# AnyDSL/rodent

Measured on AMD Instinct MI355X. Metric: Mrays/s, higher is better.
Workload: dtype f32; 1 GPU; atrium.bvh + atrium-primary.rays (1024x1024 primary rays, tmax 5000, closest hit); bvh_layout=BVH2, kernel=k_bvh2_top_auto<false,15, 255, 16, 32>, variant=top, parallelism=replicated BVH x 1, world_size=1

## Files before the change

include/rodent_traversal.h:

```cpp
#ifndef RODENT_TRAVERSAL_H
#define RODENT_TRAVERSAL_H

#include <stdint.h>
#include <stddef.h>

#ifdef __cplusplus
extern "C" {
#endif


struct Node2 {
    float   bounds[12];
    int32_t child[2];
    int32_t pad[2];
};

struct Tri1 {
    float   v0[3];  int32_t pad;
    float   e1[3];  int32_t geom_id;
    float   e2[3];  int32_t prim_id;
};

struct Node4 {
    float   bounds[6][4];
// ... 46 lines not shown
void hip_traverse_bvh2_tri1_async(int32_t dev,
        const struct Node2* nodes, const struct Tri1* tris,
        const struct Ray1* rays, struct Hit1* hits, int32_t num_rays,
        int32_t any_hit, int32_t variant, void* stream);
void hip_traverse_bvh4_tri4_async(int32_t dev,
        const struct Node4* nodes, const struct Tri4* tris,
        const struct Ray1* rays, struct Hit1* hits, int32_t num_rays,
        int32_t any_hit, int32_t variant, void* stream);
void hip_traverse_bvh8_tri4_async(int32_t dev,
        const struct Node8* nodes, const struct Tri4* tris,
        const struct Ray1* rays, struct Hit1* hits, int32_t num_rays,
        int32_t any_hit, int32_t variant, void* stream);
int32_t rodent_hip_check_errors(int32_t dev, void* stream);

uint64_t    rodent_hip_get_kernel_time(void);
int32_t     rodent_hip_device_count(void);
int32_t     rodent_hip_num_variants(int32_t bvh_width);
void        rodent_hip_phased_min_rays(int32_t rays);
void        rodent_hip_top_min_rays(int32_t rays);
void        rodent_hip_schedule_history(int32_t enable);
void        rodent_hip_ray_kind_hint(int32_t enable);
void        rodent_hip_ray_grid(int32_t width);
void        rodent_hip_octant_loops(int32_t enable);
int32_t     rodent_hip_is_lab_build(void);
const char* rodent_hip_variant_name(int32_t bvh_width, int32_t variant);
const char* rodent_hip_kernel_name(int32_t bvh_width, int32_t variant, int32_t any_hit);
const char* rodent_hip_version(void);
const char* rodent_hip_source_digest(void);
void        rodent_hip_read_stats(int32_t dev, uint64_t* out8);
void        rodent_hip_read_trace(int32_t dev, uint64_t* out);
void        rodent_hip_debug_set_perm(int32_t dev, const int32_t* device_perm);

#ifdef __cplusplus
}
#endif
#endif
```

rodent_amd/abi.py:

```python
from __future__ import annotations

import ctypes as C
import os
from pathlib import Path

import numpy as np
import torch

from . import formats as F

LAB = os.environ.get("RODENT_HIP_LAB", "0") not in ("", "0")
LIB_PATH = Path(__file__).resolve().parent / "lib" / ("librodent_hip_lab.so" if LAB else "librodent_hip.so")
if os.environ.get("RODENT_HIP_LIB"):
    LIB_PATH = Path(os.environ["RODENT_HIP_LIB"]).resolve()

SYNC_ENTRY_POINTS = [
    "amdgpu_intersect_single_ray1_bvh2_tri1", "amdgpu_occluded_single_ray1_bvh2_tri1",
    "hip_intersect_single_ray1_bvh4_tri4", "hip_occluded_single_ray1_bvh4_tri4",
    "hip_intersect_single_ray1_bvh8_tri4", "hip_occluded_single_ray1_bvh8_tri4",
]
ASYNC_ENTRY_POINTS = ["hip_traverse_bvh2_tri1_async", "hip_traverse_bvh4_tri4_async", "hip_traverse_bvh8_tri4_async"]
EXPORTS = SYNC_ENTRY_POINTS + ASYNC_ENTRY_POINTS + [
    "rodent_hip_check_errors", "rodent_hip_get_kernel_time", "rodent_hip_device_count", "rodent_hip_num_variants",
        "rodent_hip_variant_name",
    "rodent_hip_kernel_name", "rodent_hip_version", "rodent_hip_source_digest", "rodent_hip_is_lab_build", "rodent_hip_phased_min_rays",
        "rodent_hip_top_min_rays", "rodent_hip_ray_kind_hint", "rodent_hip_ray_grid", "rodent_hip_octant_loops", "rodent_hip_schedule_history",
        "rodent_hip_read_stats", "rodent_hip_read_trace", "rodent_hip_debug_set_perm",
    "rodent_hip_build_scratch_bytes", "rodent_hip_build_bvh2_tri1", "rodent_hip_build_bvh2_tri1_sync",
    "rodent_hip_build_opt_scratch_bytes", "rodent_hip_build_bvh2_tri1_opt", "rodent_hip_build_bvh2_tri1_opt_sync",
    "rodent_hip_build_split_max_refs", "rodent_hip_build_split_scratch_bytes", "rodent_hip_build_bvh2_tri1_split",
    "rodent_hip_build_bvh2_tri1_split_sync",
    "rodent_hip_refit_scratch_bytes", "rodent_hip_refit_bvh2_tri1", "rodent_hip_refit_bvh2_tri1_sync",
    "rodent_hip_refit_wide_scratch_bytes", "rodent_hip_refit_bvh4_tri4", "rodent_hip_refit_bvh4_tri4_sync",
    "rodent_hip_refit_bvh8_tri4", "rodent_hip_refit_bvh8_tri4_sync",
    "rodent_hip_collapse_scratch_bytes", "rodent_hip_collapse_bvh2_tri1", "rodent_hip_collapse_bvh2_tri1_sync",
    "rodent_hip_collapse_bounded_scratch_bytes", "rodent_hip_collapse_bvh2_tri1_bounded", "rodent_hip_collapse_bvh2_tri1_bounded_sync",
]
BLOCK_OF_WIDTH = {2: F.BVH2_TRI1, 4: F.BVH4_TRI4, 8: F.BVH8_TRI4}

_lib = None


class BuildOptions(C.Structure):
    _fields_ = [("max_leaf", C.c_int32), ("treelet_passes", C.c_int32), ("node_cost", C.c_float), ("tri_cost", C.c_float)]


class SplitOptions(C.Structure):
    _fields_ = [("budget", C.c_float), ("max_pieces", C.c_int32)]

# ... 1 lines not shown
class MissingExtension(RuntimeError):
    pass


def lib():
    global _lib
    if _lib is None:
        if not LIB_PATH.exists():
            raise MissingExtension(f"{LIB_PATH} not built: run `python -m rodent_amd.build` (needs hipcc)")
        l = C.CDLL(str(LIB_PATH))
        vp, i32 = C.c_void_p, C.c_int32
        for name in SYNC_ENTRY_POINTS:
            fn = getattr(l, name); fn.restype = None; fn.argtypes = [i32, vp, vp, vp, vp, i32]
        for name in ASYNC_ENTRY_POINTS:
            fn = getattr(l, name); fn.restype = None; fn.argtypes = [i32, vp, vp, vp, vp, i32, i32, i32, vp]
        l.rodent_hip_check_errors.restype = i32; l.rodent_hip_check_errors.argtypes = [i32, vp]
        l.rodent_hip_is_lab_build.restype = i32; l.rodent_hip_is_lab_build.argtypes = []
        l.rodent_hip_phased_min_rays.restype = None; l.rodent_hip_phased_min_rays.argtypes = [i32]
        l.rodent_hip_top_min_rays.restype = None; l.rodent_hip_top_min_rays.argtypes = [i32]
        l.rodent_hip_get_kernel_time.restype = C.c_uint64; l.rodent_hip_get_kernel_time.argtypes = []
        l.rodent_hip_ray_kind_hint.restype = None; l.rodent_hip_ray_kind_hint.argtypes = [i32]
        l.rodent_hip_ray_grid.restype = None; l.rodent_hip_ray_grid.argtypes = [i32]
        l.rodent_hip_octant_loops.restype = None; l.rodent_hip_octant_loops.argtypes = [i32]
        l.rodent_hip_schedule_history.restype = None; l.rodent_hip_schedule_history.argtypes = [i32]
        l.rodent_hip_device_count.restype = i32; l.rodent_hip_device_count.argtypes = []
        l.rodent_hip_num_variants.restype = i32; l.rodent_hip_num_variants.argtypes = [i32]
        l.rodent_hip_variant_name.restype = C.c_char_p; l.rodent_hip_variant_name.argtypes = [i32, i32]
        l.rodent_hip_kernel_name.restype = C.c_char_p; l.rodent_hip_kernel_name.argtypes = [i32, i32, i32]
        l.rodent_hip_version.restype = C.c_char_p; l.rodent_hip_version.argtypes = []
        l.rodent_hip_source_digest.restype = C.c_char_p; l.rodent_hip_source_digest.argtypes = []
        l.rodent_hip_read_trace.restype = None; l.rodent_hip_read_trace.argtypes = [i32, C.c_void_p]
        l.rodent_hip_debug_set_perm.restype = None; l.rodent_hip_debug_set_perm.argtypes = [i32, C.c_void_p]
        l.rodent_hip_read_stats.restype = None; l.rodent_hip_read_stats.argtypes = [i32, C.POINTER(C.c_uint64)]
        l.rodent_hip_build_scratch_bytes.restype = C.c_int64; l.rodent_hip_build_scratch_bytes.argtypes = [i32]
        l.rodent_hip_build_bvh2_tri1.restype = i32
        l.rodent_hip_build_bvh2_tri1.argtypes = [i32, vp, i32, vp, i32, i32, vp, vp, vp, vp, vp]
        l.rodent_hip_build_bvh2_tri1_sync.restype = i32
        l.rodent_hip_build_bvh2_tri1_sync.argtypes = [i32, vp, i32, vp, i32, i32, vp, vp, C.POINTER(i32)]
        opt = C.POINTER(BuildOptions)
        l.rodent_hip_build_opt_scratch_bytes.restype = C.c_int64; l.rodent_hip_build_opt_scratch_bytes.argtypes = [i32, opt]
        l.rodent_hip_build_bvh2_tri1_opt.restype = i32
        l.rodent_hip_build_bvh2_tri1_opt.argtypes = [i32, vp, i32, vp, i32, opt, vp, vp, vp, vp, vp]
        l.rodent_hip_build_bvh2_tri1_opt_sync.restype = i32
        l.rodent_hip_build_bvh2_tri1_opt_sync.argtypes = [i32, vp, i32, vp, i32, opt, vp, vp, C.POINTER(i32)]
        spl = C.POINTER(SplitOptions)
        l.rodent_hip_build_split_max_refs.restype = C.c_int64; l.rodent_hip_build_split_max_refs.argtypes = [i32, spl]
# ... 45 lines not shown


def kernel_name(width, variant, any_hit=False):
    return lib().rodent_hip_kernel_name(width, variant, int(any_hit)).decode()



def to_device(arr: np.ndarray, dev: int = 0):
    import torch
    if not torch.cuda.is_available():
        raise RuntimeError("rodent_amd: no GPU visible (torch.cuda.is_available() is False)")
    a = np.ascontiguousarray(arr)
    t = torch.from_numpy(a.view(np.uint8).reshape(-1).copy() if a.size else np.zeros(0, np.uint8))
    return t.to(f"cuda:{dev}")


def from_device(t, dtype: np.dtype) -> np.ndarray:
    return t.cpu().numpy().view(dtype).copy()


class DeviceBvh:

    def __init__(self, width, nodes, tris, dev=0):
        assert width in (2, 4, 8)
        self.width, self.dev = width, dev
        self.num_nodes, self.num_tris = len(nodes), len(tris)
        self.nodes = to_device(nodes, dev)
        self.tris = to_device(tris, dev)

    @classmethod
    def from_tensors(cls, width, nodes, tris, num_nodes, num_tris, dev=0):
        assert width in (2, 4, 8)
        node_dt, tri_dt = {2: (F.NODE2, F.TRI1), 4: (F.NODE4, F.TRI4), 8: (F.NODE8, F.TRI4)}[width]
        for t, count, dt in ((nodes, num_nodes, node_dt), (tris, num_tris, tri_dt)):
            if not t.is_cuda or t.numel() * t.element_size() < count * dt.itemsize or not t.is_contiguous():
                raise ValueError("DeviceBvh.from_tensors: a contiguous CUDA tensor with room for every record is needed")
        self = cls.__new__(cls)
        self.width, self.dev = width, dev
        self.num_nodes, self.num_tris = int(num_nodes), int(num_tris)
        self.nodes, self.tris = nodes, tris
        return self

    @classmethod
    def load(cls, path, width, dev=0):
        nodes, tris = F.read_bvh(path, BLOCK_OF_WIDTH[width])
        return cls(width, nodes, tris, dev)


def traverse_async(bvh: DeviceBvh, rays_dev, hits_dev, num_rays, any_hit=False, variant=0, stream=None):
    import torch
    if stream is None:
# ... 23 lines not shown
    return from_device(hits_dev, F.HIT1)[:n]


def schedule_history(enable: bool):
    lib().rodent_hip_schedule_history(int(bool(enable)))


def top_min_rays(rays: int):
    lib().rodent_hip_top_min_rays(int(rays))


def ray_kind_hint(enable: bool):
    lib().rodent_hip_ray_kind_hint(int(bool(enable)))


def ray_grid(width: int = -1):
    lib().rodent_hip_ray_grid(int(width))


def octant_loops(enable: bool = True):
    lib().rodent_hip_octant_loops(int(bool(enable)))


def check_errors(dev=0, stream=None):
    import torch
    if stream is None:
        stream = torch.cuda.current_stream(dev)
    if lib().rodent_hip_check_errors(dev, C.c_void_p(stream.cuda_stream)):
        raise RuntimeError("rodent_hip: traversal stack overflow (more than 64 entries)")


def read_stats(dev=0):
    buf = (C.c_uint64 * 8)()
    lib().rodent_hip_read_stats(dev, buf)
    return list(buf)


def read_trace(dev=0, arm_only=False):
    if arm_only:
        lib().rodent_hip_read_trace(dev, None)
        return None
    buf = np.zeros((16384, 4), np.uint64)
    lib().rodent_hip_read_trace(dev, buf.ctypes.data_as(C.c_void_p))
    return buf
```

rodent_amd/csrc/traversal.hip:

```cpp
#include <hip/hip_runtime.h>

#include <algorithm>
#include <atomic>
#include <cstdint>
#include <cstdio>
#include <cstdlib>
#include <memory>
#include <mutex>
#include <utility>
#include <vector>

#include "device_buffer.h"
#include "rodent_traversal.h"
#include "traversal_device.h"

namespace {

using namespace rodent_dev;

template <bool ANY, bool WIDE = true>
__device__ __forceinline__ bool leaf_tri1(const Tri1* __restrict__ tris, int first, RayX& ray, HitAcc& hit) {
    int j = first;
    for (;;) {
        const float4* p = WIDE ? reinterpret_cast<const float4*>(tris + j)
// ... 85 lines not shown
            report_error(ctl);
        }
    }
}

template <bool ANY>
__global__ __launch_bounds__(kWave) void k_bvh2_finish(const Node2* __restrict__ nodes, const Tri1* __restrict__ tris,
                                                        const Ray1* __restrict__ rays, Hit1* __restrict__ hits,
                                                        Ctl* ctl, const int* __restrict__ deep_list,
                                                            int* , int* phase_counters) {
    __shared__ int stack_lds[kStackCap * kWave];
    finish_launch<ANY>(nodes, tris, rays, hits, ctl, deep_list, (lds_int*)stack_lds, phase_counters, blockIdx.x, gridDim.x);
}

struct Lane {
    RayX ray;
    int top;
    lds_int* sp;
    int ray_id;
    bool found;
};
typedef const __attribute__((address_space(1))) char* gptr;
struct Bases { gptr node, tri; };
__device__ __forceinline__ Bases make_bases(const Node2* nodes, const Tri1* tris) {
    unsigned long long node_bits = reinterpret_cast<unsigned long long>(nodes - 1), tri_bits = reinterpret_cast<unsigned long long>(tris);
    asm volatile("" : "+v"(node_bits), "+v"(tri_bits));
    return Bases{(gptr)node_bits, (gptr)tri_bits};
}

typedef __attribute__((address_space(3))) float lds_float;
template <bool ANY, bool PF = false, bool TOP = false, bool LAZY = false, bool FENCE = false, bool SHARED = false, int SPILL = 0,
    int WPG = 1, int OCT = -1>
__device__ __forceinline__ void bvh2_step(Lane& L, const Bases& base, Hit1* __restrict__ hits, lds_int* sp_limit, Ctl* ctl,
    int* __restrict__ deep_list,
                                          bool prefetch = false, lds_int* pf_row = nullptr, lds_int* image = nullptr,
                                              lds_float* shared_tmax = nullptr,
                                          int* __restrict__ spill = nullptr, const RaySplat* splat = nullptr) {
    const bool is_node = L.top > 0;
    typedef float f32x4 __attribute__((ext_vector_type(4)));
    typedef int i32x2 __attribute__((ext_vector_type(2)));
    f32x4 q0, q1, q2;
    i32x2 ch;
    int popped;
    float shared_now = 0.0f;
    if constexpr (TOP && !SHARED) {
        const unsigned idx = (unsigned)(is_node ? L.top : ~L.top), stride = is_node ? (unsigned)sizeof(Node2) : (unsigned)sizeof(Tri1);
        const gptr addr = (is_node ? base.node : base.tri) + (size_t)idx * stride;
        joint_fetch(q0, q1, q2, ch, popped, L.top >= kLdsTag, (unsigned)(size_t)image + (unsigned)(L.top - kLdsTag), addr,
            addr + (is_node ? 48u : 40u), L.sp);
    } else {
        if (TOP && L.top >= kLdsTag) {
            typedef __attribute__((address_space(3))) const char* lds_bytes;
            const lds_bytes rec = (lds_bytes)image + (unsigned)(L.top - kLdsTag);
            const __attribute__((address_space(3))) f32x4* p = (const __attribute__((address_space(3))) f32x4*)rec;
            q0 = p[0]; q1 = p[1]; q2 = p[2];
            ch = *(const __attribute__((address_space(3))) i32x2*)(rec + 48);
        } else {
            const unsigned idx = (unsigned)(is_node ? L.top : ~L.top), stride = is_node ? (unsigned)sizeof(Node2) : (unsigned)sizeof(Tri1);
            const gptr addr = (is_node ? base.node : base.tri) + (size_t)idx * stride;
            const __attribute__((address_space(1))) f32x4* p = (const __attribute__((address_space(1))) f32x4*)addr;
            q0 = p[0]; q1 = p[1]; q2 = p[2];
            ch = *(const __attribute__((address_space(1))) i32x2*)(addr + (is_node ? 48u : 40u));
        }
        popped = *L.sp;
        if (SHARED) shared_now = *shared_tmax;
        asm volatile("" : "+v"(q0), "+v"(q1), "+v"(q2), "+v"(ch));
    }
    if (SHARED) {
// ... 445 lines not shown
    int want = 64;
    while (want < slots) want *= 2;
    s.spill.ensure((size_t)std::min(want, kSpillSlots) * kSpillWaveInts);
}
int persistent_groups(const DeviceState& s, int occ, int waves) {
    const int groups = ((s.num_cus * (occ / waves) + kStripes - 1) / kStripes) * kStripes;
    if ((long)groups * waves > kSpillSlots) {
        fprintf(stderr, "rodent_hip: %d x %d resident waves exceed the %d stack spill blocks\n", groups, waves, kSpillSlots); abort(); }
    return groups;
}

bool read_and_clear_error_flags(DeviceState& s, hipStream_t stream) {
    HIP_CHECK(hipStreamSynchronize(stream));
    volatile int* page = s.host_page;
    const bool raised = page[kHostErr] != 0;
    page[kHostErr] = 0;
    return raised;
}
void check_error_flag(DeviceState& s, hipStream_t stream) {
    if (read_and_clear_error_flags(s, stream)) {
        fprintf(stderr, "rodent_hip: traversal stack overflow (more than %d entries)\n", kStackCap); abort(); }
}

int mapped_node_ids(const Node2* nodes) {
    hipDeviceptr_t range_base = nullptr; size_t range_size = 0;
    if (hipMemGetAddressRange(&range_base, &range_size, (hipDeviceptr_t)nodes) != hipSuccess) { (void)hipGetLastError(); return 0; }
    const size_t bytes = (size_t)((const char*)range_base + range_size - (const char*)nodes);
    return (int)std::min<size_t>(bytes / sizeof(Node2), 0x3FFFFFFF);
}

int g_ray_grid = [] { const char* e = getenv("RODENT_HIP_RAY_GRID"); return e ? atoi(e) : -1; }();
int g_octant_loops = [] { const char* e = getenv("RODENT_HIP_OCTANT_LOOPS"); return e ? (atoi(e) ? 1 : 0) : 1; }();
int g_schedule_history = [] { const char* e = getenv("RODENT_HIP_SCHEDULE_HISTORY"); return e && atoi(e) ? 1 : 0; }();
constexpr int kFinishGroups = 256;
#define LAUNCH_ARGS DeviceState& s, const Node2* nodes, const Tri1* tris, const Ray1* rays, Hit1* hits, int n, hipStream_t stream

constexpr int kGridMinRays = 2048 * kWave;
bool reserve_single(DeviceState& s, int n, bool spill) {
    s.deep_list.ensure(n);
    spill = spill && blocks_for(n) <= kSpillSlots;
    if (spill) ensure_spill(s, blocks_for(n));
    return spill;
}
template <bool ANY, int LDS_N, int XCD, bool TR = false, int PRIO = 0> void L_single(LAUNCH_ARGS) {
    if (reserve_single(s, n, PRIO == 0 && !TR))
        hipLaunchKernelGGL((k_bvh2_single<ANY, LDS_N, XCD, false, 0, true>), dim3(blocks_for(n)), dim3(kWave), 0, stream, nodes, tris,
            rays, hits, n, s.ctl(), s.deep_list.ptr, (const int*)nullptr, s.spill.ptr, n >= kGridMinRays ? g_ray_grid : 0);
    else
        hipLaunchKernelGGL((k_bvh2_single<ANY, LDS_N, XCD, TR, PRIO>), dim3(blocks_for(n)), dim3(kWave), 0, stream, nodes, tris, rays,
            hits, n, s.ctl(), s.deep_list.ptr, (const int*)nullptr, (int*)nullptr, 0);
    hipLaunchKernelGGL((k_bvh2_finish<ANY>), dim3(kFinishGroups), dim3(kWave), 0, stream, nodes, tris, rays, hits, s.ctl(),
        s.deep_list.ptr, s.deep_stack, (int*)nullptr);
// ... 68 lines not shown
}
template <bool ANY, int LDS_N, int TOPN, int WAVES, int REFILL, int MODE = 0, bool FUSED = true,
    bool LAZY = false> void L_default(LAUNCH_ARGS) {
    const int max_id = reserve_default(s, nodes, n, WAVES);
    if (max_id == 0) { L_single<ANY, 16, 32>(s, nodes, tris, rays, hits, n, stream); return; }
    if (g_schedule_history) {
        launch_top_persist<ANY, LDS_N, TOPN, WAVES, false, false, 32, false, 0, 2>(s, nodes, tris, rays, hits, n, stream, max_id); return; }
    const int groups = persistent_groups(s, 32, WAVES);
    s.top_image_nodes = nullptr; s.order_rays = 0;
    if (s.hint_rays != rays || s.hint_n != n) { s.hint_rays = rays; s.hint_n = n; s.hint_first_id = s.launch_id + 1; }
    const int id = ++s.launch_id;
    const volatile int* kinds = s.host_kinds;
    const bool hinting = MODE == 0 && g_kind_hint;
    int* const report_to = hinting ? s.host_kinds : nullptr;
    const bool incoherent = hinting && kinds[1] >= s.hint_first_id && kinds[0] < kinds[1];
    if (incoherent) {
        hipLaunchKernelGGL((k_bvh2_top_refill<ANY, LDS_N, TOPN, WAVES, REFILL, false, false>), dim3(groups), dim3(kWave * WAVES), 0,
            stream, nodes, tris, rays, hits, n, s.ctl(), s.deep_list.ptr,
                           (const int4*)s.top_image.ptr, s.tickets.ptr, max_id, s.spill.ptr, report_to, id);
        hipLaunchKernelGGL((k_bvh2_top_finish<ANY>), dim3(1), dim3(kWave), 0, stream, nodes, tris, rays, hits, s.ctl(), s.deep_list.ptr,
            s.deep_stack, s.tickets.ptr, s.top_image.ptr, TOPN);
        return;
    }
    hipLaunchKernelGGL((k_bvh2_top_auto<ANY, LDS_N, TOPN, WAVES, REFILL, MODE, FUSED, LAZY>), dim3(groups), dim3(kWave * WAVES), 0, stream,
        nodes, tris, rays, hits, n, s.ctl(), s.deep_list.ptr,
                       s.top_image.ptr, s.tickets.ptr, max_id, s.spill.ptr, report_to, id, g_ray_grid, g_octant_loops);
    if (!FUSED) hipLaunchKernelGGL((k_bvh2_top_finish<ANY>), dim3(1), dim3(kWave), 0, stream, nodes, tris, rays, hits, s.ctl(),
        s.deep_list.ptr, s.deep_stack, s.tickets.ptr, s.top_image.ptr, TOPN);
}

template <bool ANY, int LDS_N, int TOPN, int WAVES, int REFILL, bool ADAPT = false, bool FENCE = false> void L_top_refill(LAUNCH_ARGS) {
    if (top_kernel_ids(nodes, n) == 0) { L_single<ANY, 16, 32>(s, nodes, tris, rays, hits, n, stream); return; }
    const int groups = persistent_groups(s, 32, WAVES);
    s.deep_list.ensure(n);
    ensure_top_buffers(s);
    s.top_image_nodes = nullptr;
    ensure_spill(s, groups * WAVES);
    hipLaunchKernelGGL((k_bvh2_top_refill<ANY, LDS_N, TOPN, WAVES, REFILL, ADAPT, FENCE>), dim3(groups), dim3(kWave * WAVES), 0, stream,
        nodes, tris, rays, hits, n, s.ctl(), s.deep_list.ptr,
                       (const int4*)s.top_image.ptr, s.tickets.ptr, mapped_node_ids(nodes), s.spill.ptr, (int*)nullptr, 0);
    hipLaunchKernelGGL((k_bvh2_top_finish<ANY>), dim3(1), dim3(kWave), 0, stream, nodes, tris, rays, hits, s.ctl(), s.deep_list.ptr,
        s.deep_stack, s.tickets.ptr, s.top_image.ptr, TOPN);
}



template <bool ANY, int LDS_N> void L_sorted(LAUNCH_ARGS) {
    s.deep_list.ensure(n);
    ensure_sort_buffers(s, n);
// ... 195 lines not shown
    timed_sync_call(dev, num_rays, nullptr,
        [&](DeviceState& s) { launch_wide(8, false, s, nodes, tris, rays, hits, num_rays, default_variant(8), nullptr); });
}
void hip_occluded_single_ray1_bvh8_tri4(int32_t dev, const Node8* nodes, const Tri4* tris, const Ray1* rays, Hit1* hits, int32_t num_rays) {
    timed_sync_call(dev, num_rays, nullptr,
        [&](DeviceState& s) { launch_wide(8, true, s, nodes, tris, rays, hits, num_rays, default_variant(8), nullptr); });
}

int32_t rodent_hip_device_count(void) {
    int count = 0;
    if (hipGetDeviceCount(&count) != hipSuccess) return 0;
    return count;
}
int32_t rodent_hip_num_variants(int32_t bvh_width) {
    if (bvh_width == 2) return kNumVariants2;
    int count = 0; wide_variants(bvh_width, &count); return count;
}
const char* rodent_hip_variant_name(int32_t bvh_width, int32_t variant) {
    if (bvh_width == 2) return variant >= 0 && variant < kNumVariants2 ? kVariants2[variant].name : "";
    int count = 0; const VariantW* t = wide_variants(bvh_width, &count);
    return variant >= 0 && variant < count ? t[variant].name : "";
}
const char* rodent_hip_kernel_name(int32_t bvh_width, int32_t variant, int32_t any_hit) {
    if (bvh_width == 2) return variant >= 0 && variant < kNumVariants2 ? kVariants2[variant].kernel[any_hit ? 1 : 0] : "";
    int count = 0; const VariantW* t = wide_variants(bvh_width, &count);
    return variant >= 0 && variant < count ? t[variant].kernel[any_hit ? 1 : 0] : "";
}
void rodent_hip_phased_min_rays(int32_t rays) { g_phased_min_rays = rays < 0 ? 4096 * kWave : rays; }
void rodent_hip_debug_set_perm(int32_t dev, const int32_t* device_perm) { device_state(dev).debug_perm = device_perm; }
void rodent_hip_schedule_history(int32_t enable) { g_schedule_history = enable ? 1 : 0; }
void rodent_hip_top_min_rays(int32_t rays) { g_top_min_rays = rays < 0 ? kTopMinRays : rays; }
void rodent_hip_ray_kind_hint(int32_t enable) { g_kind_hint = enable ? 1 : 0; }
void rodent_hip_ray_grid(int32_t width) { g_ray_grid = width; }
void rodent_hip_octant_loops(int32_t enable) { g_octant_loops = enable ? 1 : 0; }
int32_t rodent_hip_is_lab_build(void) {
#ifdef RODENT_HIP_LAB
    return 1;
#else
    return 0;
#endif
}
void rodent_hip_read_trace(int32_t dev, uint64_t* out) {
    DeviceState& s = device_state(dev);
    HIP_CHECK(hipSetDevice(dev));
    HIP_CHECK(hipDeviceSynchronize());
    std::lock_guard<std::mutex> launching(s.mutex);
    const size_t bytes = 16384 * 4 * sizeof(uint64_t);
    if (!s.trace.ptr) {
        s.trace.ensure(16384 * 4, 0);
        HIP_CHECK(hipMemcpy(&s.ctl()->trace, &s.trace.ptr, sizeof(void*), hipMemcpyHostToDevice));
    }
    if (out) HIP_CHECK(hipMemcpy(out, s.trace.ptr, bytes, hipMemcpyDeviceToHost));
    HIP_CHECK(hipMemset(s.trace.ptr, 0, bytes));
}
void rodent_hip_read_stats(int32_t dev, uint64_t* out) {
    DeviceState& s = device_state(dev);
    HIP_CHECK(hipSetDevice(dev));
// ... 8 lines not shown
```

rodent_amd/csrc/traversal_device.h:

```cpp
#pragma once
#include <hip/hip_runtime.h>
#include <cstdint>
#include "rodent_traversal.h"

namespace rodent_dev {

constexpr int   kWave = 64;
constexpr int   kStackCap = 64;
constexpr float kFltMax = 3.4028234664e+38f;

struct RayX {
    float ox, oy, oz, dx, dy, dz, idx, idy, idz, iox, ioy, ioz, tmin, tmax;
};

__device__ __forceinline__ float prodsign(float x, float y) {
    return __int_as_float(__float_as_int(x) ^ (__float_as_int(y) & (int)0x80000000u));
}
__device__ __forceinline__ float safe_rcp(float x) {
    return (fabsf(x) < 1e-8f) ? prodsign(kFltMax, x) : 1.0f / x;
}
__device__ __forceinline__ float dot3(float ax, float ay, float az, float bx, float by, float bz) {
    return fmaf(az, bz, fmaf(ay, by, ax * bx));
}
__device__ __forceinline__ float cross_x(float ax, float ay, float az, float bx, float by, float bz) { return fmaf(ay, bz, -(az * by)); }
// ... 150 lines not shown
    asm volatile("s_mov_b64 %[save], exec\n\t"
                 "s_andn2_b64 exec, exec, %[lm]\n\t"
                 "s_cbranch_execz .Ljoint_a_%=\n\t"
                 "global_load_dwordx4 %[q1], %[a], off offset:16\n\t"
                 "global_load_dwordx4 %[q0], %[a], off\n\t"
                 "global_load_dwordx4 %[q2], %[a], off offset:32\n\t"
                 "global_load_dwordx2 %[ch], %[ac], off\n"
                 ".Ljoint_a_%=:\n\t"
                 "s_and_b64 exec, %[save], %[lm]\n\t"
                 "s_cbranch_execz .Ljoint_b_%=\n\t"
                 "ds_read_b128 %[q0], %[l]\n\t"
                 "ds_read_b128 %[q1], %[l] offset:16\n\t"
                 "ds_read_b128 %[q2], %[l] offset:32\n\t"
                 "ds_read_b64 %[ch], %[l] offset:48\n"
                 ".Ljoint_b_%=:\n\t"
                 "s_mov_b64 exec, %[save]\n\t"
                 "ds_read_b32 %[pop], %[sp]\n\t"
                 "s_waitcnt vmcnt(0) lgkmcnt(0)"
                 : [q0] "=&v"(q0), [q1] "=&v"(q1), [q2] "=&v"(q2), [ch] "=&v"(ids), [pop] "=&v"(popped), [save] "=&s"(save)
                 : [a] "v"(addr), [ac] "v"(addr_ids), [l] "v"(lds_addr), [sp] "v"(sp_addr), [lm] "s"(lds_mask)
                 : "memory", "scc");
}

__device__ __forceinline__ void wave_lds_sync() { __builtin_amdgcn_fence(__ATOMIC_SEQ_CST, "wavefront"); __builtin_amdgcn_wave_barrier(); }
__device__ __forceinline__ void build_top_image(const Node2* __restrict__ nodes, int4* __restrict__ image, int capacity,
    lds_int* slot_node ) {
    const int lane = threadIdx.x;
    if (lane == 0) slot_node[0] = 1;
    wave_lds_sync();
    int begin = 0, end = 1;
    while (begin < end) {
        int next = end;
        for (int first = begin; first < end; first += kWave) {
            const int slot = first + lane;
            const bool on = slot < end;
            int4 r0 = {}, r1 = {}, r2 = {}, r3 = {};
            if (on) { const int4* p = reinterpret_cast<const int4*>(nodes + (slot_node[slot] - 1)); r0 = p[0]; r1 = p[1]; r2 = p[2];
                r3 = p[3]; }
            const bool in0 = on && r3.x > 0, in1 = on && r3.y > 0;
            const unsigned long long m0 = __ballot(in0), m1 = __ballot(in1), below = (1ull << lane) - 1ull;
            const int s0 = next + __popcll(m0 & below), s1 = next + __popcll(m0) + __popcll(m1 & below);
            if (in0 && s0 < capacity) { slot_node[s0] = r3.x; r3.x = kLdsTag + s0 * (int)sizeof(Node2); }
            if (in1 && s1 < capacity) { slot_node[s1] = r3.y; r3.y = kLdsTag + s1 * (int)sizeof(Node2); }
            next = min(capacity, next + __popcll(m0) + __popcll(m1));
            if (on) { r3.z = slot_node[slot]; r3.w = 0; int4* q = image + 4 * slot; q[0] = r0; q[1] = r1; q[2] = r2; q[3] = r3; }
        }
// ... 7 lines not shown
```

rodent_amd/csrc/traversal_top.h:

```cpp
#pragma once

template <int TOPN>
__global__ __launch_bounds__(kWave) void k_bvh2_top_image(const Node2* __restrict__ nodes, int4* __restrict__ image) {
    __shared__ int slot_node[TOPN];
    build_top_image(nodes, image, TOPN, (lds_int*)slot_node);
}

template <bool ANY>
__global__ __launch_bounds__(kWave) void k_bvh2_top_finish(const Node2* __restrict__ nodes, const Tri1* __restrict__ tris,
                                                            const Ray1* __restrict__ rays, Hit1* __restrict__ hits,
                                                            Ctl* ctl, const int* __restrict__ deep_list, int* deep_stack, int* tickets,
                                                            int4* __restrict__ image, int capacity) {
    __shared__ int stack_lds[kStackCap * kWave];
    static_assert(kStackCap * kWave >= kMaxTopNodes, "slot table");
    const bool stale = ctl->reserved != 0;
    finish_launch<ANY>(nodes, tris, rays, hits, ctl, deep_list, (lds_int*)stack_lds, tickets, blockIdx.x, gridDim.x);
    if (stale && blockIdx.x == 0) {
        build_top_image(nodes, image, capacity, (lds_int*)stack_lds);
        if (threadIdx.x == 0) ctl->reserved = 0;
    }
}


__device__ __forceinline__ int stripe_rank(int wave) { return wave * ((int)gridDim.x / kStripes) + (int)blockIdx.x / kStripes; }
// ... 282 lines not shown

template <bool ANY, int LDS_N, int TOPN, int WAVES, int REFILL, bool ADAPT = false, bool FENCE = false>
__global__ __launch_bounds__(kWave * WAVES, 32 / WAVES) void k_bvh2_top_refill(const Node2* __restrict__ nodes,
    const Tri1* __restrict__ tris,
                                                                    const Ray1* __restrict__ rays, Hit1* __restrict__ hits, int n,
                                                                    Ctl* ctl, int* __restrict__ deep_list,
                                                                        const int4* __restrict__ top_image, int* __restrict__ tickets,
                                                                        int max_id,
                                                                    int* spill, int* host_kinds, int launch_id) {
    top_refill_body<ANY, LDS_N, TOPN, WAVES, REFILL, ADAPT, FENCE>(nodes, tris, rays, hits, n, ctl, deep_list, top_image, tickets, max_id,
        spill, host_kinds, launch_id);
}

__device__ __forceinline__ int chunk_octant(const Lane& L) {
    const RayX& r = L.ray;
    const auto negative = [](float x) { return (int)((unsigned)__float_as_int(x) >> 31); };
    const int oct = negative(r.idx) | (negative(r.idy) << 1) | (negative(r.idz) << 2);
    const auto finite3 = [](float x, float y, float z) { return __builtin_isfinite(x) && __builtin_isfinite(y) && __builtin_isfinite(z); };
    const bool finite = finite3(r.ox, r.oy, r.oz) && finite3(r.dx, r.dy, r.dz) && finite3(r.idx, r.idy, r.idz)
        && finite3(r.iox, r.ioy, r.ioz);
    const int first = __builtin_amdgcn_readfirstlane(oct);
    return __ballot(L.ray_id >= 0 && !(finite && oct == first)) == 0ull ? first : -1;
}
template <bool ANY, bool LAZY, int LDS_N, int WAVES, int OCT>
__device__ __forceinline__ void trace_chunk(Lane& L, const Bases& base, Hit1* __restrict__ hits, lds_int* sp_limit, Ctl* ctl,
    int* __restrict__ deep_list, lds_int* image, int* __restrict__ spill, const RaySplat* splat) {
    while (__ballot(L.top != 0)) {
        if (L.top != 0) bvh2_step<ANY, false, true, LAZY, false, false, LDS_N, WAVES, OCT>(L, base, hits, sp_limit, ctl, deep_list,
            false, nullptr, image, nullptr, spill, splat);
    }
}

template <bool ANY, int LDS_N, int TOPN, int WAVES, int REFILL,
    int MODE = 0 ,
    bool FUSED = true , bool LAZY = false>
__global__ __launch_bounds__(kWave * WAVES) __attribute__((amdgpu_waves_per_eu(8, 8))) void
    k_bvh2_top_auto(const Node2* __restrict__ nodes, const Tri1* __restrict__ tris,
                                                                  const Ray1* __restrict__ rays, Hit1* __restrict__ hits, int n,
                                                                  Ctl* ctl, int* __restrict__ deep_list, int4* __restrict__ top_image,
                                                                      int* __restrict__ tickets, int max_id,
                                                                  int* spill, int* host_kinds, int launch_id, int grid_w,
                                                                      int octant_loops) {
    constexpr int kStackInts = WAVES * (LDS_N + 1) * kWave, kGroupRays = 32 * kWave;
    static_assert((kStackInts + TOPN * 16) * 4 * (32 / WAVES) <= 160 * 1024, "32 waves per CU must fit their stacks and images in LDS");
    __shared__ __attribute__((aligned(16))) int lds_raw[kStackInts + TOPN * 16];
    const int lane = threadIdx.x % kWave, wave = threadIdx.x / kWave;
    lds_int* col = (lds_int*)lds_raw + wave * (LDS_N + 1) * kWave + lane;
    lds_int* image = (lds_int*)lds_raw + kStackInts;
    const int root = stage_top_image<TOPN, kWave * WAVES>(nodes, (const int4*)top_image, image, (lds_int*)lds_raw, ctl, max_id)
        ? kLdsTag : 1;
    if (root != 1 && threadIdx.x == 0 && blockIdx.x == 0) atomicAdd(&ctl->stats[6], 1ull);
    const int stripe = blockIdx.x % kStripes, stripe_waves = (gridDim.x / kStripes) * WAVES;
    int* counter = tickets + stripe * kCounterStride;
    const auto ray_of = [&](int t) { return ((t / kGroupRays) * kStripes + stripe) * kGroupRays + t % kGroupRays; };
    lds_int* const sp_limit = col + LDS_N * kWave;
    const Bases base = make_bases(nodes, tris);
    int t = stripe_rank(wave) * kWave;
    bool coherent = MODE != 2;
    if (MODE == 0 && ray_of(t) < n) {
        const int r = ray_of(t + lane);
        const float4* p = reinterpret_cast<const float4*>(rays + (r < n ? r : ray_of(t)));
        const float4 o = p[0], d = p[1];
        if (grid_w < 0) grid_w = detect_ray_grid(rays, n);
        coherent = wave_rays_coherent(o.x, o.y, o.z, d.x, d.y, d.z, r < n);
        if (wave == 0) report_ray_kind(host_kinds, launch_id, coherent);
    }
    if (!coherent && threadIdx.x == 0 && blockIdx.x == 0) atomicAdd(&ctl->stats[5], 1ull);
    grid_w = __builtin_amdgcn_readfirstlane(grid_w > 0 && (grid_w & 7) == 0 ? grid_w : 0);
    const int tiled_rays = tiled_ray_count(grid_w, n);
    if (grid_w > 0 && threadIdx.x == 0 && blockIdx.x == 0) atomicAdd(&ctl->stats[2], (unsigned long long)grid_w);
    if (MODE == 1 || (MODE == 0 && coherent)) {
        for (;;) {
            int first_ray = ray_of(t);
            if (first_ray >= n) break;
            int r = ray_of(t + lane);
            if (first_ray < tiled_rays) r = tile_ray(first_ray, lane, grid_w);
            Lane L = start_lane<LAZY>(rays, hits, r < n ? r : -1, first_ray, window_base<LDS_N>(sp_limit));
            if (L.top != 0) L.top = root;
            const int oct = octant_loops ? chunk_octant(L) : -1;
            if (oct >= 0 && lane == 0 && blockIdx.x == 0) atomicAdd(&ctl->stats[3], 1ull);
            int arm = oct;
            const RaySplat splat = splat_ray(L.ray);
            static_assert(LDS_N > 0, "bvh2_step<SPILL = LDS_N>: the ray id is only the hit record's index");
            const int ray_id = L.ray_id;
            Hit1* lane_hit = hits + ray_id;
            asm volatile("" : "+v"(lane_hit));
            L.ray_id = 0;
#define RODENT_TRACE_CHUNK(OCT) if (arm == OCT) trace_chunk<ANY, LAZY, LDS_N, WAVES, OCT>(L, base, lane_hit, sp_limit, ctl, deep_list, image, spill, \
                &splat); \
            asm volatile("" : "+s"(arm))
            RODENT_TRACE_CHUNK(0); RODENT_TRACE_CHUNK(1); RODENT_TRACE_CHUNK(2); RODENT_TRACE_CHUNK(3);
            RODENT_TRACE_CHUNK(4); RODENT_TRACE_CHUNK(5); RODENT_TRACE_CHUNK(6); RODENT_TRACE_CHUNK(7);
#undef RODENT_TRACE_CHUNK
            trace_chunk<ANY, LAZY, LDS_N, WAVES, kAnyOctantSplat>(L, base, lane_hit, sp_limit, ctl, deep_list, image, spill, &splat);
            L.ray_id = ray_id;
            if (LAZY) finish_lane_reg(L, rays, hits);
            int t_next = 0;
            if (lane == 0) t_next = atomicAdd(counter, kWave);
            t = stripe_waves * kWave + __builtin_amdgcn_readfirstlane(t_next);
        }
    } else if (MODE != 1) {
        const auto ray_at = [&](int pos) { return pos < tiled_rays ? tile_ray_at(pos, grid_w) : pos; };
        Lane L;
        {
            const int r = ray_at(ray_of(t + lane));
            L = start_lane<LAZY>(rays, hits, r < n ? r : -1, 0, col);
            if (L.top != 0) L.top = root;
        }
        bool more = true;
        for (;;) {
            const unsigned long long live = __ballot(L.top != 0);
            if (more && __popcll(live) <= kWave - REFILL) {
                const int want = kWave - __popcll(live);
                int first = 0;
                if (lane == 0) first = atomicAdd(counter, want);
                first = stripe_waves * kWave + __builtin_amdgcn_readfirstlane(first);
                more = ray_of(first) < n;
                if (L.top == 0) {
                    if (LAZY) { finish_lane_reg(L, rays, hits); L.ray_id = -1; }
                    const int pos = ray_of(first + __popcll(~live & ((1ull << lane) - 1ull)));
                    if (pos < n) {
                        const int rr = ray_at(pos);
                        L = start_lane<LAZY>(rays, hits, rr, rr, col);
                        L.top = root;
                    }
                }
                continue;
            }
            if (live == 0) break;
            if (L.top != 0) bvh2_step<ANY, false, true, LAZY, false, false, LDS_N, WAVES>(L, base, hits, sp_limit, ctl, deep_list, false,
                nullptr, image, nullptr, spill);
        }
        if (LAZY) finish_lane_reg(L, rays, hits);
    }
    if (!FUSED) return;
    __syncthreads();
    if (threadIdx.x == 0) lds_raw[0] = __hip_atomic_fetch_add(&ctl->counter, 1, __ATOMIC_RELAXED,
        __HIP_MEMORY_SCOPE_AGENT) == (int)gridDim.x - 1;
    __syncthreads();
    if (!lds_raw[0] || wave != 0) return;
    const int deep = __hip_atomic_load(&ctl->deep_count, __ATOMIC_RELAXED, __HIP_MEMORY_SCOPE_AGENT);
    if (deep > 0) __threadfence();
    const bool stale = __hip_atomic_load(&ctl->reserved, __ATOMIC_RELAXED, __HIP_MEMORY_SCOPE_AGENT) != 0;
    finish_launch<ANY>(nodes, tris, rays, hits, ctl, deep_list, (lds_int*)lds_raw, tickets, 0, 1, deep);
    if (stale) {
        build_top_image(nodes, top_image, TOPN, (lds_int*)lds_raw);
        if (lane == 0) ctl->reserved = 0;
    }
}
```

Measured before the change: 6370 Mrays/s.

## Fetch BVH nodes and triangles via 32-bit offsets from one shared scalar base

Places nodes and triangles in one device buffer and, when both fit within a 4 GiB span, launches a kernel variant that addresses every record as a scalar base plus a 32-bit VGPR offset computed with a 24-bit multiply-add. The aim is to replace per-lane 64-bit address arithmetic and the two separate VGPR base pointers in the joint LDS/global fetch, saving VALU work and registers. It adds a host-side eligibility check, a second kernel instantiation, and a stats counter write. The risk is that the tighter id limits make it fall back to the old path on larger scenes.

```diff
diff --git a/include/rodent_traversal.h b/include/rodent_traversal.h
--- a/include/rodent_traversal.h
+++ b/include/rodent_traversal.h
@@ -92,6 +92,8 @@
 void        rodent_hip_ray_kind_hint(int32_t enable);
 void        rodent_hip_ray_grid(int32_t width);
 void        rodent_hip_octant_loops(int32_t enable);
+void        rodent_hip_record_offsets(int32_t enable);
+int32_t     rodent_hip_record_offsets_ok(uint64_t nodes, uint64_t node_bytes, uint64_t tris, uint64_t tri_bytes);
 int32_t     rodent_hip_is_lab_build(void);
 const char* rodent_hip_variant_name(int32_t bvh_width, int32_t variant);
 const char* rodent_hip_kernel_name(int32_t bvh_width, int32_t variant, int32_t any_hit);
diff --git a/rodent_amd/abi.py b/rodent_amd/abi.py
--- a/rodent_amd/abi.py
+++ b/rodent_amd/abi.py
@@ -25,6 +25,7 @@
         "rodent_hip_variant_name",
     "rodent_hip_kernel_name", "rodent_hip_version", "rodent_hip_source_digest", "rodent_hip_is_lab_build", "rodent_hip_phased_min_rays",
         "rodent_hip_top_min_rays", "rodent_hip_ray_kind_hint", "rodent_hip_ray_grid", "rodent_hip_octant_loops", "rodent_hip_schedule_history",
+        "rodent_hip_record_offsets", "rodent_hip_record_offsets_ok",
         "rodent_hip_read_stats", "rodent_hip_read_trace", "rodent_hip_debug_set_perm",
     "rodent_hip_build_scratch_bytes", "rodent_hip_build_bvh2_tri1", "rodent_hip_build_bvh2_tri1_sync",
     "rodent_hip_build_opt_scratch_bytes", "rodent_hip_build_bvh2_tri1_opt", "rodent_hip_build_bvh2_tri1_opt_sync",
@@ -72,6 +73,8 @@
         l.rodent_hip_ray_kind_hint.restype = None; l.rodent_hip_ray_kind_hint.argtypes = [i32]
         l.rodent_hip_ray_grid.restype = None; l.rodent_hip_ray_grid.argtypes = [i32]
         l.rodent_hip_octant_loops.restype = None; l.rodent_hip_octant_loops.argtypes = [i32]
+        l.rodent_hip_record_offsets.restype = None; l.rodent_hip_record_offsets.argtypes = [i32]
+        l.rodent_hip_record_offsets_ok.restype = i32; l.rodent_hip_record_offsets_ok.argtypes = [C.c_uint64] * 4
         l.rodent_hip_schedule_history.restype = None; l.rodent_hip_schedule_history.argtypes = [i32]
         l.rodent_hip_device_count.restype = i32; l.rodent_hip_device_count.argtypes = []
         l.rodent_hip_num_variants.restype = i32; l.rodent_hip_num_variants.argtypes = [i32]
@@ -163,11 +166,19 @@
 class DeviceBvh:
 
     def __init__(self, width, nodes, tris, dev=0):
+        import torch
         assert width in (2, 4, 8)
         self.width, self.dev = width, dev
         self.num_nodes, self.num_tris = len(nodes), len(tris)
-        self.nodes = to_device(nodes, dev)
-        self.tris = to_device(tris, dev)
+        if not torch.cuda.is_available():
+            raise RuntimeError("rodent_amd: no GPU visible (torch.cuda.is_available() is False)")
+        nb, tb = (np.ascontiguousarray(a).view(np.uint8).reshape(-1) if len(a) else np.zeros(0, np.uint8) for a in (nodes, tris))
+        start = (len(nb) + 255) // 256 * 256
+        host = np.zeros(start + len(tb), np.uint8)
+        host[:len(nb)] = nb
+        host[start:] = tb
+        self.buffer = torch.from_numpy(host).to(f"cuda:{dev}")
+        self.nodes, self.tris = self.buffer[:len(nb)], self.buffer[start:]
 
     @classmethod
     def from_tensors(cls, width, nodes, tris, num_nodes, num_tris, dev=0):
@@ -237,6 +248,14 @@
     lib().rodent_hip_octant_loops(int(bool(enable)))
 
 
+def record_offsets(enable: bool = True):
+    lib().rodent_hip_record_offsets(int(bool(enable)))
+
+
+def record_offsets_ok(nodes: int, node_bytes: int, tris: int, tri_bytes: int) -> bool:
+    return bool(lib().rodent_hip_record_offsets_ok(int(nodes), int(node_bytes), int(tris), int(tri_bytes)))
+
+
 def check_errors(dev=0, stream=None):
     import torch
     if stream is None:
diff --git a/rodent_amd/csrc/traversal.hip b/rodent_amd/csrc/traversal.hip
--- a/rodent_amd/csrc/traversal.hip
+++ b/rodent_amd/csrc/traversal.hip
@@ -131,6 +131,17 @@
 };
 typedef const __attribute__((address_space(1))) char* gptr;
 struct Bases { gptr node, tri; };
+struct RecordOffsets { gptr base; int d_node, d_tri; };
+__device__ __forceinline__ RecordOffsets make_offsets(const char* base, int d_node, int d_tri) {
+    unsigned long long base_bits = reinterpret_cast<unsigned long long>(base);
+    asm volatile("" : "+v"(d_node), "+v"(d_tri), "+s"(base_bits));
+    return RecordOffsets{(gptr)base_bits, d_node, d_tri};
+}
+constexpr int kOffsetIdBits = 23;
+__device__ __forceinline__ unsigned record_offset(int top, bool is_node, const RecordOffsets& o) {
+    static_assert(sizeof(Node2) == 64 && sizeof(Tri1) == 48 && (1 << kOffsetIdBits) <= (1 << 23), "strides and ids fit v_mad_i32_i24");
+    return (unsigned)(__mul24(top, is_node ? (int)sizeof(Node2) : -(int)sizeof(Tri1)) + (is_node ? o.d_node : o.d_tri));
+}
 __device__ __forceinline__ Bases make_bases(const Node2* nodes, const Tri1* tris) {
     unsigned long long node_bits = reinterpret_cast<unsigned long long>(nodes - 1), tri_bits = reinterpret_cast<unsigned long long>(tris);
     asm volatile("" : "+v"(node_bits), "+v"(tri_bits));
@@ -139,12 +150,13 @@
 
 typedef __attribute__((address_space(3))) float lds_float;
 template <bool ANY, bool PF = false, bool TOP = false, bool LAZY = false, bool FENCE = false, bool SHARED = false, int SPILL = 0,
-    int WPG = 1, int OCT = -1>
+    int WPG = 1, int OCT = -1, bool OFFS = false>
 __device__ __forceinline__ void bvh2_step(Lane& L, const Bases& base, Hit1* __restrict__ hits, lds_int* sp_limit, Ctl* ctl,
     int* __restrict__ deep_list,
                                           bool prefetch = false, lds_int* pf_row = nullptr, lds_int* image = nullptr,
                                               lds_float* shared_tmax = nullptr,
-                                          int* __restrict__ spill = nullptr, const RaySplat* splat = nullptr) {
+                                          int* __restrict__ spill = nullptr, const RaySplat* splat = nullptr,
+                                              const RecordOffsets* offs = nullptr) {
     const bool is_node = L.top > 0;
     typedef float f32x4 __attribute__((ext_vector_type(4)));
     typedef int i32x2 __attribute__((ext_vector_type(2)));
@@ -152,7 +164,11 @@
     i32x2 ch;
     int popped;
     float shared_now = 0.0f;
-    if constexpr (TOP && !SHARED) {
+    static_assert(!OFFS || (TOP && !SHARED && !PF), "the offset form exists for the joint fetch of the LDS-image kernels");
+    if constexpr (OFFS) {
+        joint_fetch(q0, q1, q2, ch, popped, L.top >= kLdsTag, (unsigned)(size_t)image + (unsigned)(L.top - kLdsTag), offs->base,
+            record_offset(L.top, is_node, *offs), is_node, L.sp);
+    } else if constexpr (TOP && !SHARED) {
         const unsigned idx = (unsigned)(is_node ? L.top : ~L.top), stride = is_node ? (unsigned)sizeof(Node2) : (unsigned)sizeof(Tri1);
         const gptr addr = (is_node ? base.node : base.tri) + (size_t)idx * stride;
         joint_fetch(q0, q1, q2, ch, popped, L.top >= kLdsTag, (unsigned)(size_t)image + (unsigned)(L.top - kLdsTag), addr,
@@ -644,12 +660,23 @@
         fprintf(stderr, "rodent_hip: traversal stack overflow (more than %d entries)\n", kStackCap); abort(); }
 }
 
-int mapped_node_ids(const Node2* nodes) {
+size_t mapped_bytes(const void* p) {
     hipDeviceptr_t range_base = nullptr; size_t range_size = 0;
-    if (hipMemGetAddressRange(&range_base, &range_size, (hipDeviceptr_t)nodes) != hipSuccess) { (void)hipGetLastError(); return 0; }
-    const size_t bytes = (size_t)((const char*)range_base + range_size - (const char*)nodes);
-    return (int)std::min<size_t>(bytes / sizeof(Node2), 0x3FFFFFFF);
-}
+    if (hipMemGetAddressRange(&range_base, &range_size, (hipDeviceptr_t)p) != hipSuccess) { (void)hipGetLastError(); return 0; }
+    return (size_t)((const char*)range_base + range_size - (const char*)p);
+}
+int mapped_node_ids(const Node2* nodes) { return (int)std::min<size_t>(mapped_bytes(nodes) / sizeof(Node2), 0x3FFFFFFF); }
+
+bool record_offsets_ok(uint64_t nodes, uint64_t node_bytes, uint64_t tris, uint64_t tri_bytes) {
+    constexpr uint64_t kMaxIds = (1ull << kOffsetIdBits) - 1, kSpan = 1ull << 32;
+    if (node_bytes == 0 || tri_bytes == 0) return false;
+    if (node_bytes > ~nodes || tri_bytes > ~tris) return false;
+    if (node_bytes / sizeof(Node2) > kMaxIds || tri_bytes / sizeof(Tri1) > kMaxIds) return false;
+    const uint64_t lo = std::min(nodes, tris), end = std::max(nodes + node_bytes, tris + tri_bytes);
+    return end - lo < kSpan;
+}
+int g_record_offsets = [] { const char* e = getenv("RODENT_HIP_RECORD_OFFSETS"); return e ? (atoi(e) ? 1 : 0) : 1; }();
+std::atomic<int> g_last_record_form{-1};
 
 int g_ray_grid = [] { const char* e = getenv("RODENT_HIP_RAY_GRID"); return e ? atoi(e) : -1; }();
 int g_octant_loops = [] { const char* e = getenv("RODENT_HIP_OCTANT_LOOPS"); return e ? (atoi(e) ? 1 : 0) : 1; }();
@@ -764,9 +791,22 @@
             s.deep_stack, s.tickets.ptr, s.top_image.ptr, TOPN);
         return;
     }
-    hipLaunchKernelGGL((k_bvh2_top_auto<ANY, LDS_N, TOPN, WAVES, REFILL, MODE, FUSED, LAZY>), dim3(groups), dim3(kWave * WAVES), 0, stream,
-        nodes, tris, rays, hits, n, s.ctl(), s.deep_list.ptr,
-                       s.top_image.ptr, s.tickets.ptr, max_id, s.spill.ptr, report_to, id, g_ray_grid, g_octant_loops);
+    const uint64_t node_bits = (uint64_t)(uintptr_t)nodes, tri_bits = (uint64_t)(uintptr_t)tris;
+    const bool offsets = g_record_offsets && record_offsets_ok(node_bits, (uint64_t)max_id * sizeof(Node2), tri_bits, mapped_bytes(tris));
+    g_last_record_form.store(offsets ? 1 : 0, std::memory_order_relaxed);
+    if (offsets) {
+        const uint64_t lo = std::min(node_bits, tri_bits);
+        const int d_node = (int)((uint32_t)(node_bits - lo) - (uint32_t)sizeof(Node2)),
+            d_tri = (int)((uint32_t)(tri_bits - lo) - (uint32_t)sizeof(Tri1));
+        hipLaunchKernelGGL((k_bvh2_top_auto<ANY, LDS_N, TOPN, WAVES, REFILL, MODE, FUSED, LAZY, true>), dim3(groups), dim3(kWave * WAVES), 0,
+            stream, nodes, tris, rays, hits, n, s.ctl(), s.deep_list.ptr,
+                           s.top_image.ptr, s.tickets.ptr, max_id, s.spill.ptr, report_to, id, g_ray_grid, g_octant_loops,
+                               (const char*)(uintptr_t)lo, d_node, d_tri);
+    } else
+    hipLaunchKernelGGL((k_bvh2_top_auto<ANY, LDS_N, TOPN, WAVES, REFILL, MODE, FUSED, LAZY, false>), dim3(groups), dim3(kWave * WAVES), 0,
+        stream, nodes, tris, rays, hits, n, s.ctl(), s.deep_list.ptr,
+                       s.top_image.ptr, s.tickets.ptr, max_id, s.spill.ptr, report_to, id, g_ray_grid, g_octant_loops,
+                           (const char*)nullptr, 0, 0);
     if (!FUSED) hipLaunchKernelGGL((k_bvh2_top_finish<ANY>), dim3(1), dim3(kWave), 0, stream, nodes, tris, rays, hits, s.ctl(),
         s.deep_list.ptr, s.deep_stack, s.tickets.ptr, s.top_image.ptr, TOPN);
 }
@@ -1008,6 +1048,13 @@
     return variant >= 0 && variant < count ? t[variant].name : "";
 }
 const char* rodent_hip_kernel_name(int32_t bvh_width, int32_t variant, int32_t any_hit) {
+    if (bvh_width == 2 && variant == 0) {
+        const int last = g_last_record_form.load(std::memory_order_relaxed);
+        static const char* const names[2][2] = {
+            {"k_bvh2_top_auto<false,15,255,16,32,0,true,false,false>", "k_bvh2_top_auto<false,15,255,16,32,0,true,false,true>"},
+            {"k_bvh2_top_auto<true,15,255,16,32,0,true,false,false>", "k_bvh2_top_auto<true,15,255,16,32,0,true,false,true>"}};
+        return names[any_hit ? 1 : 0][(last < 0 ? g_record_offsets : last) ? 1 : 0];
+    }
     if (bvh_width == 2) return variant >= 0 && variant < kNumVariants2 ? kVariants2[variant].kernel[any_hit ? 1 : 0] : "";
     int count = 0; const VariantW* t = wide_variants(bvh_width, &count);
     return variant >= 0 && variant < count ? t[variant].kernel[any_hit ? 1 : 0] : "";
@@ -1019,6 +1066,10 @@
 void rodent_hip_ray_kind_hint(int32_t enable) { g_kind_hint = enable ? 1 : 0; }
 void rodent_hip_ray_grid(int32_t width) { g_ray_grid = width; }
 void rodent_hip_octant_loops(int32_t enable) { g_octant_loops = enable ? 1 : 0; }
+void rodent_hip_record_offsets(int32_t enable) { g_record_offsets = enable ? 1 : 0; g_last_record_form.store(-1, std::memory_order_relaxed); }
+int32_t rodent_hip_record_offsets_ok(uint64_t nodes, uint64_t node_bytes, uint64_t tris, uint64_t tri_bytes) {
+    return record_offsets_ok(nodes, node_bytes, tris, tri_bytes) ? 1 : 0;
+}
 int32_t rodent_hip_is_lab_build(void) {
 #ifdef RODENT_HIP_LAB
     return 1;
diff --git a/rodent_amd/csrc/traversal_device.h b/rodent_amd/csrc/traversal_device.h
--- a/rodent_amd/csrc/traversal_device.h
+++ b/rodent_amd/csrc/traversal_device.h
@@ -196,6 +196,35 @@
                  : "memory", "scc");
 }
 
+__device__ __forceinline__ void joint_fetch(vf4& q0, vf4& q1, vf4& q2, vi2& ids, int& popped, bool in_lds, unsigned lds_addr, gbytes base,
+    unsigned off, bool is_node, lds_int* sp) {
+    const unsigned long long lds_mask = __ballot(in_lds), node_mask = __ballot(is_node);
+    const unsigned sp_addr = (unsigned)(size_t)sp;
+    unsigned long long save;
+    asm volatile("s_mov_b64 %[save], exec\n\t"
+                 "s_andn2_b64 exec, exec, %[lm]\n\t"
+                 "s_cbranch_execz .Ljoint_e_%=\n\t"
+                 "global_load_dwordx4 %[q1], %[o], %[sb] offset:16\n\t"
+                 "global_load_dwordx4 %[q0], %[o], %[sb]\n\t"
+                 "global_load_dwordx4 %[q2], %[o], %[sb] offset:32\n\t"
+                 "s_and_b64 exec, exec, %[nm]\n\t"
+                 "global_load_dwordx2 %[ch], %[o], %[sb] offset:48\n"
+                 ".Ljoint_e_%=:\n\t"
+                 "s_and_b64 exec, %[save], %[lm]\n\t"
+                 "s_cbranch_execz .Ljoint_f_%=\n\t"
+                 "ds_read_b128 %[q0], %[l]\n\t"
+                 "ds_read_b128 %[q1], %[l] offset:16\n\t"
+                 "ds_read_b128 %[q2], %[l] offset:32\n\t"
+                 "ds_read_b64 %[ch], %[l] offset:48\n"
+                 ".Ljoint_f_%=:\n\t"
+                 "s_mov_b64 exec, %[save]\n\t"
+                 "ds_read_b32 %[pop], %[sp]\n\t"
+                 "s_waitcnt vmcnt(0) lgkmcnt(0)"
+                 : [q0] "=&v"(q0), [q1] "=&v"(q1), [q2] "=&v"(q2), [ch] "=&v"(ids), [pop] "=&v"(popped), [save] "=&s"(save)
+                 : [o] "v"(off), [sb] "s"(base), [l] "v"(lds_addr), [sp] "v"(sp_addr), [lm] "s"(lds_mask), [nm] "s"(node_mask)
+                 : "memory", "scc");
+}
+
 __device__ __forceinline__ void wave_lds_sync() { __builtin_amdgcn_fence(__ATOMIC_SEQ_CST, "wavefront"); __builtin_amdgcn_wave_barrier(); }
 __device__ __forceinline__ void build_top_image(const Node2* __restrict__ nodes, int4* __restrict__ image, int capacity,
     lds_int* slot_node ) {
diff --git a/rodent_amd/csrc/traversal_top.h b/rodent_amd/csrc/traversal_top.h
--- a/rodent_amd/csrc/traversal_top.h
+++ b/rodent_amd/csrc/traversal_top.h
@@ -328,25 +328,27 @@
     const int first = __builtin_amdgcn_readfirstlane(oct);
     return __ballot(L.ray_id >= 0 && !(finite && oct == first)) == 0ull ? first : -1;
 }
-template <bool ANY, bool LAZY, int LDS_N, int WAVES, int OCT>
+template <bool ANY, bool LAZY, int LDS_N, int WAVES, int OCT, bool OFFS>
 __device__ __forceinline__ void trace_chunk(Lane& L, const Bases& base, Hit1* __restrict__ hits, lds_int* sp_limit, Ctl* ctl,
-    int* __restrict__ deep_list, lds_int* image, int* __restrict__ spill, const RaySplat* splat) {
+    int* __restrict__ deep_list, lds_int* image, int* __restrict__ spill, const RaySplat* splat, const RecordOffsets* offs) {
     while (__ballot(L.top != 0)) {
-        if (L.top != 0) bvh2_step<ANY, false, true, LAZY, false, false, LDS_N, WAVES, OCT>(L, base, hits, sp_limit, ctl, deep_list,
-            false, nullptr, image, nullptr, spill, splat);
+        if (L.top != 0) bvh2_step<ANY, false, true, LAZY, false, false, LDS_N, WAVES, OCT, OFFS>(L, base, hits, sp_limit, ctl, deep_list,
+            false, nullptr, image, nullptr, spill, splat, offs);
     }
 }
 
 template <bool ANY, int LDS_N, int TOPN, int WAVES, int REFILL,
     int MODE = 0 ,
-    bool FUSED = true , bool LAZY = false>
+    bool FUSED = true , bool LAZY = false,
+    bool OFFS = false >
 __global__ __launch_bounds__(kWave * WAVES) __attribute__((amdgpu_waves_per_eu(8, 8))) void
     k_bvh2_top_auto(const Node2* __restrict__ nodes, const Tri1* __restrict__ tris,
                                                                   const Ray1* __restrict__ rays, Hit1* __restrict__ hits, int n,
                                                                   Ctl* ctl, int* __restrict__ deep_list, int4* __restrict__ top_image,
                                                                       int* __restrict__ tickets, int max_id,
                                                                   int* spill, int* host_kinds, int launch_id, int grid_w,
-                                                                      int octant_loops) {
+                                                                      int octant_loops,
+                                                                  const char* record_base, int d_node, int d_tri) {
     constexpr int kStackInts = WAVES * (LDS_N + 1) * kWave, kGroupRays = 32 * kWave;
     static_assert((kStackInts + TOPN * 16) * 4 * (32 / WAVES) <= 160 * 1024, "32 waves per CU must fit their stacks and images in LDS");
     __shared__ __attribute__((aligned(16))) int lds_raw[kStackInts + TOPN * 16];
@@ -356,11 +358,13 @@
     const int root = stage_top_image<TOPN, kWave * WAVES>(nodes, (const int4*)top_image, image, (lds_int*)lds_raw, ctl, max_id)
         ? kLdsTag : 1;
     if (root != 1 && threadIdx.x == 0 && blockIdx.x == 0) atomicAdd(&ctl->stats[6], 1ull);
+    if (threadIdx.x == 0 && blockIdx.x == 0) atomicAdd(&ctl->stats[OFFS ? 1 : 0], 1ull);
     const int stripe = blockIdx.x % kStripes, stripe_waves = (gridDim.x / kStripes) * WAVES;
     int* counter = tickets + stripe * kCounterStride;
     const auto ray_of = [&](int t) { return ((t / kGroupRays) * kStripes + stripe) * kGroupRays + t % kGroupRays; };
     lds_int* const sp_limit = col + LDS_N * kWave;
-    const Bases base = make_bases(nodes, tris);
+    const Bases base = OFFS ? Bases{nullptr, nullptr} : make_bases(nodes, tris);
+    const RecordOffsets offsets = make_offsets(record_base, d_node, d_tri);
     int t = stripe_rank(wave) * kWave;
     bool coherent = MODE != 2;
     if (MODE == 0 && ray_of(t) < n) {
@@ -389,16 +393,18 @@
             const RaySplat splat = splat_ray(L.ray);
             static_assert(LDS_N > 0, "bvh2_step<SPILL = LDS_N>: the ray id is only the hit record's index");
             const int ray_id = L.ray_id;
-            Hit1* lane_hit = hits + ray_id;
-            asm volatile("" : "+v"(lane_hit));
+            unsigned long long hit_bits = reinterpret_cast<unsigned long long>(hits + ray_id);
+            asm volatile("" : "+v"(hit_bits));
+            Hit1* lane_hit = (Hit1*)(__attribute__((address_space(1))) Hit1*)hit_bits;
             L.ray_id = 0;
-#define RODENT_TRACE_CHUNK(OCT) if (arm == OCT) trace_chunk<ANY, LAZY, LDS_N, WAVES, OCT>(L, base, lane_hit, sp_limit, ctl, deep_list, image, spill, \
-                &splat); \
+#define RODENT_TRACE_CHUNK(OCT) if (arm == OCT) trace_chunk<ANY, LAZY, LDS_N, WAVES, OCT, OFFS>(L, base, lane_hit, sp_limit, ctl, deep_list, image, \
+                spill, &splat, &offsets); \
             asm volatile("" : "+s"(arm))
             RODENT_TRACE_CHUNK(0); RODENT_TRACE_CHUNK(1); RODENT_TRACE_CHUNK(2); RODENT_TRACE_CHUNK(3);
             RODENT_TRACE_CHUNK(4); RODENT_TRACE_CHUNK(5); RODENT_TRACE_CHUNK(6); RODENT_TRACE_CHUNK(7);
 #undef RODENT_TRACE_CHUNK
-            trace_chunk<ANY, LAZY, LDS_N, WAVES, kAnyOctantSplat>(L, base, lane_hit, sp_limit, ctl, deep_list, image, spill, &splat);
+            trace_chunk<ANY, LAZY, LDS_N, WAVES, kAnyOctantSplat, OFFS>(L, base, lane_hit, sp_limit, ctl, deep_list, image, spill, &splat,
+                &offsets);
             L.ray_id = ray_id;
             if (LAZY) finish_lane_reg(L, rays, hits);
             int t_next = 0;
@@ -434,8 +440,8 @@
                 continue;
             }
             if (live == 0) break;
-            if (L.top != 0) bvh2_step<ANY, false, true, LAZY, false, false, LDS_N, WAVES>(L, base, hits, sp_limit, ctl, deep_list, false,
-                nullptr, image, nullptr, spill);
+            if (L.top != 0) bvh2_step<ANY, false, true, LAZY, false, false, LDS_N, WAVES, -1, OFFS>(L, base, hits, sp_limit, ctl, deep_list,
+                false, nullptr, image, nullptr, spill, nullptr, &offsets);
         }
         if (LAZY) finish_lane_reg(L, rays, hits);
     }
```

After: 6768 Mrays/s, median of 6. 6.3% higher.
